# JohnLonginotto/uq

Measured on NVIDIA B200. Metric: fastq_to_uq_encode_reads_per_s, higher is better.
Workload: dtype u8

## Files before the change

uq_b200/csrc/common.cuh:

```cuda
#pragma once
#include <cuda_runtime.h>
#include <stdint.h>
#include <stdio.h>
#include <string.h>
#include <string>
#include <vector>
#include <map>
#include "../../include/uqb200.h"

#define UQB_SM_COUNT 148

struct uqb_timer_rec { const char* name; cudaEvent_t a, b; uint64_t bytes; };
struct uqb_timer_tot { uint64_t launches = 0; double ms = 0; uint64_t bytes = 0; };

struct uqb_arena {
    unsigned long long base = 0;
    uint64_t reserved = 0;
    uint64_t mapped = 0;
    uint64_t granularity = 0;
    std::map<uint64_t, uint64_t> free_by_off;
    std::map<uint64_t, uint64_t> used;
    std::vector<unsigned long long> handles;
    std::vector<std::pair<uint64_t, uint64_t>> chunks;
};
// ... 5 lines not shown
    bool own_stream = false;
    cudaStream_t copy_stream = nullptr;
    char err[512] = {0};
    uint64_t launches = 0;
    uint64_t bytes_in_use = 0;
    int sm_count = UQB_SM_COUNT;
    std::vector<const void*> copies_in_flight;
    unsigned side_ctas_per_sm = 0;
    void* pinned = nullptr;
    size_t pinned_bytes = 0;
    bool timing = false;
    std::vector<uqb_timer_rec> pending;
    std::vector<cudaEvent_t> free_events;
    std::map<std::string, uqb_timer_tot> totals;
    cudaEvent_t span_a = nullptr, span_b = nullptr;
};

struct uqb_array {
    void* d = nullptr;
    uint64_t n = 0;
    uint32_t width = 0;
    bool owned = true;
    uint64_t* key0 = nullptr;
    uint64_t nbytes() const { return n * (uint64_t)width; }
};

struct uqb_qcol {
    int64_t* val = nullptr;
    uint32_t* span = nullptr;
    uint32_t* rank = nullptr;
    uint32_t* first_occ = nullptr;
    uint8_t* dict = nullptr;
    uint64_t dict_count = 0;
    uint32_t dict_width = 0;
};

struct uqb_fastq {
    const uint8_t* d = nullptr;
    uint64_t n = 0;
    bool owned = false;
    uint64_t* line_off = nullptr;
    uint64_t n_lines = 0, n_reads = 0;
    uint64_t total_bases = 0;
    uint8_t* ref_name = nullptr;
    uint32_t ref_len = 0;
    uint64_t rbase = 0;
    uint8_t* names = nullptr;
    uint32_t name_pitch = 0;
    uint64_t names_cap = 0;
    uint64_t line_cap = 0;
    void* scan_acc = nullptr;
    bool streamed = false;
    uqb_stats* cached_stats = nullptr;
    uint32_t prefix_len = 0, suffix_len = 0, ncols = 0;
    std::vector<uqb_qcol> qcols;
};

int uqb_fail(uqb_ctx* ctx, const char* fmt, ...);

#define UQB_CUDA(expr)                                                                       \
    do {                                                                                     \
        cudaError_t _e = (expr);                                                             \
        if (_e != cudaSuccess)                                                               \
            return uqb_fail(ctx, "%s:%d %s -> %s", __FILE__, __LINE__, #expr, cudaGetErrorString(_e)); \
    } while (0)

#define UQB_TRY(expr)                                                                        \
    do {                                                                                     \
        int _r = (expr);                                                                     \
        if (_r != 0) return _r;                                                              \
    } while (0)

int uqb_dalloc(uqb_ctx* ctx, void** p, size_t nbytes);
int uqb_dfree(uqb_ctx* ctx, void* p, size_t nbytes);
int uqb_new_array(uqb_ctx* ctx, uint64_t n, uint32_t width, uqb_array** out);
int uqb_adopt_array(uqb_ctx* ctx, void* d, uint64_t n, uint32_t width, uqb_array** out);
int uqb_pinned(uqb_ctx* ctx, size_t nbytes, void** out);
int uqb_readback(uqb_ctx* ctx, void* host, const void* dev, size_t nbytes);

template <typename T>
static inline int uqb_dalloc_t(uqb_ctx* ctx, T** p, size_t count) {
    return uqb_dalloc(ctx, (void**)p, count * sizeof(T));
}

void uqb_timer_begin(uqb_ctx* ctx, const char* name, uint64_t bytes);
void uqb_timer_end(uqb_ctx* ctx);
void uqb_timer_add_bytes(uqb_ctx* ctx, uint64_t bytes);

#define UQB_LAUNCH(kernel, grid, block, smem, ...) UQB_LAUNCH_B(0, kernel, grid, block, smem, __VA_ARGS__)
#define UQB_LAUNCH_B(abytes, kernel, grid, block, smem, ...)                                 \
    do {                                                                                     \
        uqb_timer_begin(ctx, #kernel, (uint64_t)(abytes));                                   \
        kernel<<<(grid), (block), (smem), ctx->stream>>>(__VA_ARGS__);                       \
        uqb_timer_end(ctx);                                                                  \
        ctx->launches++;                                                                     \
        UQB_CUDA(cudaGetLastError());                                                        \
    } while (0)

static inline unsigned uqb_blocks(uint64_t n, unsigned per_block) {
    uint64_t b = (n + per_block - 1) / per_block;
    if (b == 0) b = 1;
    return (unsigned)b;
}

static inline unsigned uqb_grid(uqb_ctx* ctx, uint64_t n, unsigned per_block, unsigned waves = 8) {
    uint64_t need = (n + per_block - 1) / per_block;
    uint64_t cap = (uint64_t)ctx->sm_count * waves;
    if (need < 1) need = 1;
    return (unsigned)(need < cap ? need : cap);
}

#ifdef __CUDACC__
__device__ __forceinline__ unsigned lane_id() { return threadIdx.x & 31u; }

__device__ __forceinline__ uint64_t load_be64(const uint8_t* p, uint32_t avail) {
    uint64_t v = 0;
#pragma unroll
    for (int i = 0; i < 8; i++) {
        uint64_t b = (uint32_t)i < avail ? (uint64_t)__ldg(p + i) : 0ull;
        v = (v << 8) | b;
    }
    return v;
}

__device__ __forceinline__ void atomic_min_i64(int64_t* addr, int64_t v) {
    atomicMin((long long*)addr, (long long)v);
}
__device__ __forceinline__ void atomic_max_i64(int64_t* addr, int64_t v) {
    atomicMax((long long*)addr, (long long)v);
}
#endif

#define UQB_SPLIT_TILE (256 * 64)
int uqb_split_count_tiles(uqb_ctx* ctx, const uint8_t* d, uint64_t n_end, uint64_t tile0, uint64_t ntiles, uint32_t* counts);
int uqb_split_write_tiles(uqb_ctx* ctx, const uint8_t* d, uint64_t n_end, uint64_t tile0, uint64_t ntiles, uint64_t line_base,
                          const uint64_t* bases, uint64_t* line_off);
int uqb_split_set_first(uqb_ctx* ctx, uint64_t* line_off);
int uqb_copy_stream(uqb_ctx* ctx, cudaStream_t* out);
int uqb_scan_file(uqb_ctx* ctx, uqb_fastq* fq, bool* done);
int uqb_scan_release(uqb_ctx* ctx, uqb_fastq* fq);

int uqb_scan_u32(uqb_ctx* ctx, const uint32_t* d_in, uint32_t* d_out, uint64_t n, uint32_t* d_total);
int uqb_scan_u32_to_u64(uqb_ctx* ctx, const uint32_t* d_in, uint64_t* d_out, uint64_t n, uint64_t* d_total);

struct uqb_sortbuf {
    uint64_t* key[2] = {nullptr, nullptr};
    uint32_t* aux[2] = {nullptr, nullptr};
    uint32_t* val[2] = {nullptr, nullptr};
    int cur = 0;
    uint64_t cap = 0;
};
int uqb_sortbuf_alloc(uqb_ctx* ctx, uqb_sortbuf* sb, uint64_t n, bool with_aux);
int uqb_sortbuf_free(uqb_ctx* ctx, uqb_sortbuf* sb);
int uqb_radix_sort(uqb_ctx* ctx, uqb_sortbuf* sb, uint64_t n, bool use_aux, const uint64_t* key_first = nullptr);
int uqb_scatter_pairs_u32(uqb_ctx* ctx, const uint32_t* idx, const uint32_t* val, uint64_t n, uint32_t* out);

int uqb_sort_rows_impl(uqb_ctx* ctx, const uint8_t* rows, uint64_t n, uint32_t width,
                       uint32_t** d_perm, uint32_t** d_gid_sorted, uint64_t* n_unique, const uint64_t* key0 = nullptr,
                       uint64_t** sorted_keys = nullptr);
```

uq_b200/csrc/prims.cu:

```cuda
#include "common.cuh"

#define PR_THREADS 256
#define PR_ITEMS 16
#define PR_TILE (PR_THREADS * PR_ITEMS)

template <typename T>
__device__ __forceinline__ T block_exclusive_scan(T v, T* total_out) {
    __shared__ T warp_tot[PR_THREADS / 32];
    unsigned lane = lane_id(), w = threadIdx.x >> 5;
    T incl = v;
#pragma unroll
    for (int o = 1; o < 32; o <<= 1) {
        T t = __shfl_up_sync(0xffffffffu, incl, o);
        if (lane >= (unsigned)o) incl += t;
    }
    if (lane == 31) warp_tot[w] = incl;
    __syncthreads();
    T wbase = 0, tot = 0;
#pragma unroll
    for (int i = 0; i < PR_THREADS / 32; i++) {
        T t = warp_tot[i];
        if ((unsigned)i < w) wbase += t;
        tot += t;
    }
// ... 486 lines not shown
    const uint64_t tile0 = (uint64_t)tile * PR_TILE;
    const uint64_t warp0 = tile0 + (uint64_t)w * (32 * RS_ITEMS);
    const uint32_t ntile = (uint32_t)((n - tile0 < PR_TILE) ? (n - tile0) : PR_TILE);
    uint64_t key[RS_ITEMS];
    uint32_t val[RS_ITEMS];
#pragma unroll
    for (int j = 0; j < RS_ITEMS; j++) {
        const uint64_t idx = warp0 + (uint64_t)j * 32 + lane;
        key[j] = 0; val[j] = 0;
        if (idx < n) {
            key[j] = kin[idx];
            val[j] = vin ? vin[idx] : (uint32_t)idx;
        }
    }
    uint32_t rk[RS_ITEMS];
#pragma unroll
    for (int j = 0; j < RS_ITEMS; j++) {
        const uint64_t idx = warp0 + (uint64_t)j * 32 + lane;
        const bool valid = idx < n;
        uint32_t d = 256u;
        if (valid) d = (uint32_t)((key[j] >> shift) & 255ull);
        const unsigned m = __match_any_sync(0xffffffffu, d);
        const unsigned r = __popc(m & ((1u << lane) - 1u));
        const int leader = __ffs(m) - 1;
        uint32_t old = 0;
        if (valid && (int)lane == leader) {
            old = S->whist[w][d];
            S->whist[w][d] = old + __popc(m);
        }
        old = __shfl_sync(0xffffffffu, old, leader);
        rk[j] = (d << 16) | (old + r);
        if (next_shift >= 0 && valid) atomicAdd(&S->nhist[(uint32_t)((key[j] >> next_shift) & 255ull)], 1u);
        __syncwarp();
    }
    __syncthreads();
    uint32_t tot = 0, incl = 0;
    if (tid < 256) {
#pragma unroll
        for (int w2 = 0; w2 < RS_WARPS; w2++) {
            const uint32_t c = S->whist[w2][tid];
            S->whist[w2][tid] = tot;
            tot += c;
        }
        uint32_t* st = status + (uint64_t)tile * 256 + tid;
        __threadfence();
        os_st(st, (tile == 0 ? OS_FLAG_INC : OS_FLAG_AGG) | tot);
        incl = tot;
#pragma unroll
        for (int o = 1; o < 32; o <<= 1) {
            const uint32_t t = __shfl_up_sync(0xffffffffu, incl, o);
            if (lane >= (unsigned)o) incl += t;
        }
        if (lane == 31) S->wtot[w] = incl;
        if (next_shift >= 0 && S->nhist[tid]) atomicAdd(&ghist_next[tid], S->nhist[tid]);
    }
    __syncthreads();
    if (tid < 256) {
        uint32_t wb = 0;
#pragma unroll
        for (int i = 0; i < 8; i++) if ((unsigned)i < w) wb += S->wtot[i];
        const uint32_t start = wb + incl - tot;
        S->dstart[tid] = start;
        const uint32_t gh = __ldg(ghist + tid);
        uint32_t gin = gh;
#pragma unroll
        for (int o = 1; o < 32; o <<= 1) {
            const uint32_t t = __shfl_up_sync(0xffffffffu, gin, o);
            if (lane >= (unsigned)o) gin += t;
        }
        if (lane == 31) S->gtot[w] = gin;
        asm volatile("bar.sync 1, 256;" ::: "memory");
        uint32_t gb = 0;
#pragma unroll
        for (int i = 0; i < 8; i++) if ((unsigned)i < w) gb += S->gtot[i];
        const uint32_t gexcl = gb + gin - gh;
        uint32_t before = 0;
        if (tile) {
            uint32_t j = tile - 1;
            while (true) {
                uint32_t v = os_ld(status + (uint64_t)j * 256 + tid);
                while ((v & (OS_FLAG_AGG | OS_FLAG_INC)) == 0) { __nanosleep(32); v = os_ld(status + (uint64_t)j * 256 + tid); }
                before += v & OS_COUNT;
                if ((v & OS_FLAG_INC) || j == 0) break;
                j--;
            }
            __threadfence();
            os_st(status + (uint64_t)tile * 256 + tid, OS_FLAG_INC | (before + tot));
        }
        S->gbase[tid] = gexcl + before - start;
    }
    __syncthreads();
#pragma unroll
    for (int j = 0; j < RS_ITEMS; j++) {
        const uint64_t idx = warp0 + (uint64_t)j * 32 + lane;
        if (idx < n) {
            const uint32_t d = rk[j] >> 16;
            const uint32_t slot = S->dstart[d] + S->whist[w][d] + (rk[j] & 0xffffu);
            S->key[slot] = key[j];
            S->val[slot] = val[j];
        }
    }
    __syncthreads();
    for (uint32_t i = tid; i < ntile; i += RS_THREADS) {
        const uint64_t k = S->key[i];
        const uint32_t d = (uint32_t)((k >> shift) & 255ull);
        const uint32_t pos = S->gbase[d] + i;
        kout[pos] = k;
        vout[pos] = S->val[i];
    }
}

int uqb_sortbuf_alloc(uqb_ctx* ctx, uqb_sortbuf* sb, uint64_t n, bool with_aux) {
    sb->cap = n;
    sb->cur = 0;
    for (int i = 0; i < 2; i++) {
        UQB_TRY(uqb_dalloc_t(ctx, &sb->key[i], n));
        UQB_TRY(uqb_dalloc_t(ctx, &sb->val[i], n + 16));
        if (with_aux) UQB_TRY(uqb_dalloc_t(ctx, &sb->aux[i], n));
    }
    return 0;
}

int uqb_sortbuf_free(uqb_ctx* ctx, uqb_sortbuf* sb) {
    for (int i = 0; i < 2; i++) {
        UQB_TRY(uqb_dfree(ctx, sb->key[i], sb->cap * 8)); sb->key[i] = nullptr;
        UQB_TRY(uqb_dfree(ctx, sb->val[i], sb->cap * 4)); sb->val[i] = nullptr;
        if (sb->aux[i]) { UQB_TRY(uqb_dfree(ctx, sb->aux[i], sb->cap * 4)); sb->aux[i] = nullptr; }
    }
    return 0;
}

static int plan_windows(uint64_t varying, int nbits, int* shifts) {
    int cnt = 0;
    int b = 0;
    while (b < nbits) {
        if ((varying >> b) & 1ull) {
            shifts[cnt++] = b;
            b += 8;
        } else {
            b++;
        }
    }
    return cnt;
}

__global__ void __launch_bounds__(256) k_key_iota(const uint64_t* __restrict__ kin, uint64_t* __restrict__ kout, uint32_t* __restrict__ vout, uint64_t n) {
    for (uint64_t i = (uint64_t)blockIdx.x * blockDim.x + threadIdx.x; i < n; i += (uint64_t)gridDim.x * blockDim.x) { kout[i] = kin[i]; vout[i] = (uint32_t)i; }
}

#define MSD_MIN_N (1u << 20)

struct msd_counts { uint32_t nseg, nbuck, ntiles, pad; };

struct bs_stage {
    uint32_t whist[RS_WARPS][256];
    uint32_t dstart[256];
    uint32_t wtot[8];
    unsigned long long or64, and64;
    uint64_t key[PR_TILE];
    uint32_t val[PR_TILE];
};

__global__ void __launch_bounds__(RS_THREADS, 2) k_bucket_sort(const uint64_t* __restrict__ kin, const uint32_t* __restrict__ vin,
                                                              uint64_t* __restrict__ kout, uint32_t* __restrict__ vout,
                                                              const uint2* __restrict__ segs) {
    extern __shared__ __align__(16) uint8_t bs_raw[];
    bs_stage* S = reinterpret_cast<bs_stage*>(bs_raw);
    const unsigned tid = threadIdx.x, w = tid >> 5, lane = tid & 31u;
    const uint2 seg = segs[blockIdx.x];
    const uint64_t base = seg.x;
    const uint32_t m = seg.y;
    if (tid == 0) { S->or64 = 0ull; S->and64 = ~0ull; }
    __syncthreads();
    unsigned long long o64 = 0ull, a64 = ~0ull;
    for (uint32_t i = tid; i < m; i += RS_THREADS) {
        const uint64_t k = kin[base + i];
        S->key[i] = k;
        S->val[i] = vin[base + i];
        o64 |= k; a64 &= k;
    }
#pragma unroll
    for (int o = 16; o > 0; o >>= 1) {
        o64 |= __shfl_xor_sync(0xffffffffu, o64, o);
        a64 &= __shfl_xor_sync(0xffffffffu, a64, o);
    }
    if (lane == 0) { atomicOr(&S->or64, o64); atomicAnd(&S->and64, a64); }
    __syncthreads();
    uint64_t vary = S->or64 ^ S->and64;
    while (vary) {
        const int shift = __ffsll((long long)vary) - 1;
        vary = shift + 8 >= 64 ? 0ull : vary & (~0ull << (shift + 8));
        uint64_t key[RS_ITEMS];
        uint32_t val[RS_ITEMS], rk[RS_ITEMS];
#pragma unroll
        for (int j = 0; j < RS_ITEMS; j++) {
            const uint32_t i = w * (32 * RS_ITEMS) + j * 32 + lane;
            key[j] = i < m ? S->key[i] : 0ull;
            val[j] = i < m ? S->val[i] : 0u;
        }
        for (unsigned i = tid; i < RS_WARPS * 256; i += RS_THREADS) (&S->whist[0][0])[i] = 0;
        __syncthreads();
#pragma unroll
        for (int j = 0; j < RS_ITEMS; j++) {
            const uint32_t i = w * (32 * RS_ITEMS) + j * 32 + lane;
            const bool valid = i < m;
            const uint32_t d = valid ? (uint32_t)((key[j] >> shift) & 255ull) : 256u;
            const unsigned mm = __match_any_sync(0xffffffffu, d);
            const unsigned r = __popc(mm & ((1u << lane) - 1u));
            const int leader = __ffs(mm) - 1;
            uint32_t old = 0;
            if (valid && (int)lane == leader) {
                old = S->whist[w][d];
                S->whist[w][d] = old + __popc(mm);
            }
            old = __shfl_sync(0xffffffffu, old, leader);
            rk[j] = (d << 16) | (old + r);
            __syncwarp();
        }
        __syncthreads();
        uint32_t tot = 0, incl = 0;
        if (tid < 256) {
#pragma unroll
            for (int w2 = 0; w2 < RS_WARPS; w2++) {
                const uint32_t c = S->whist[w2][tid];
                S->whist[w2][tid] = tot;
                tot += c;
            }
            incl = tot;
#pragma unroll
            for (int o = 1; o < 32; o <<= 1) {
                const uint32_t t = __shfl_up_sync(0xffffffffu, incl, o);
                if (lane >= (unsigned)o) incl += t;
            }
            if (lane == 31) S->wtot[w] = incl;
        }
        __syncthreads();
        if (tid < 256) {
            uint32_t wb = 0;
#pragma unroll
            for (int i = 0; i < 8; i++) if ((unsigned)i < w) wb += S->wtot[i];
            S->dstart[tid] = wb + incl - tot;
        }
        __syncthreads();
#pragma unroll
        for (int j = 0; j < RS_ITEMS; j++) {
            const uint32_t i = w * (32 * RS_ITEMS) + j * 32 + lane;
            if (i < m) {
                const uint32_t d = rk[j] >> 16;
                const uint32_t slot = S->dstart[d] + S->whist[w][d] + (rk[j] & 0xffffu);
                S->key[slot] = key[j];
                S->val[slot] = val[j];
            }
        }
        __syncthreads();
    }
    for (uint32_t i = tid; i < m; i += RS_THREADS) {
        kout[base + i] = S->key[i];
        vout[base + i] = S->val[i];
    }
}

__global__ void __launch_bounds__(256) k_msd_plan(const uint32_t* __restrict__ goff, const msd_bucket* __restrict__ buckets, int last,
                                                 msd_counts* __restrict__ cnt, uint2* __restrict__ segs, msd_bucket* __restrict__ next,
                                                 uint32_t* __restrict__ next_tile_bucket) {
    __shared__ uint32_t st[257];
    __shared__ uint2 lseg[256], lover[256];
    __shared__ uint32_t nls, nlo, sbase, obase, t0s;
    const unsigned tid = threadIdx.x;
    const msd_bucket b = buckets[blockIdx.x];
    const uint64_t h0 = (uint64_t)b.t0 * 256;
    st[tid] = b.start + (goff[h0 + (uint64_t)tid * b.nt] - goff[h0]);
    if (tid == 0) st[256] = b.start + b.size;
    __syncthreads();
    if (last) {
        const uint32_t s = st[tid + 1] - st[tid], nch = (s + PR_TILE - 1) / PR_TILE;
        if (nch) {
            const uint32_t at = atomicAdd(&cnt->nseg, nch);
            for (uint32_t k = 0; k < nch; k++) segs[at + k] = make_uint2(st[tid] + k * PR_TILE, min((uint32_t)PR_TILE, s - k * PR_TILE));
        }
        return;
    }
    if (tid == 0) {
        uint32_t ns = 0, no = 0, cs = 0, cn = 0;
        for (int d = 0; d < 256; d++) {
            const uint32_t s = st[d + 1] - st[d];
            if (s == 0) continue;
            if (s > PR_TILE) {
                if (cn) { lseg[ns++] = make_uint2(cs, cn); cn = 0; }
                lover[no++] = make_uint2(st[d], s);
            } else {
                if (cn + s > PR_TILE) { lseg[ns++] = make_uint2(cs, cn); cn = 0; }
                if (cn == 0) cs = st[d];
                cn += s;
            }
        }
        if (cn) lseg[ns++] = make_uint2(cs, cn);
        nls = ns; nlo = no;
        sbase = ns ? atomicAdd(&cnt->nseg, ns) : 0u;
        obase = no ? atomicAdd(&cnt->nbuck, no) : 0u;
    }
    __syncthreads();
    for (uint32_t i = tid; i < nls; i += 256) segs[sbase + i] = lseg[i];
    for (uint32_t k = 0; k < nlo; k++) {
        const uint2 o = lover[k];
        const uint32_t nt = (o.y + PR_TILE - 1) / PR_TILE;
        if (tid == 0) {
            t0s = atomicAdd(&cnt->ntiles, nt);
            next[obase + k] = msd_bucket{o.x, o.y, t0s, nt};
        }
        __syncthreads();
        for (uint32_t t = tid; t < nt; t += 256) next_tile_bucket[t0s + t] = obase + k;
        __syncthreads();
    }
}

static int msd_shift(uint64_t vary, int below) {
    const uint64_t v = below >= 64 ? vary : vary & ((1ull << below) - 1);
    if (!v) return -1;
    const int hi = 63 - __builtin_clzll(v);
    return hi >= 7 ? hi - 7 : 0;
}

static int msd_sort(uqb_ctx* ctx, uqb_sortbuf* sb, uint64_t n, const uint64_t* key_first, uint64_t vary) {
    const uint32_t nblk = (uint32_t)((n + PR_TILE - 1) / PR_TILE);
    const uint64_t cap_b = n / PR_TILE + 1, cap_t = nblk + cap_b;
    const int fin = sb->cur ^ 1;
    msd_bucket* bk[2];
    uint32_t* tb[2];
    msd_counts* cnt;
    UQB_TRY(uqb_dalloc_t(ctx, &bk[0], cap_b));
    UQB_TRY(uqb_dalloc_t(ctx, &bk[1], cap_b));
    UQB_TRY(uqb_dalloc_t(ctx, &tb[0], cap_t));
    UQB_TRY(uqb_dalloc_t(ctx, &tb[1], cap_t));
    UQB_TRY(uqb_dalloc_t(ctx, &cnt, 1));
    const msd_bucket all = {0u, (uint32_t)n, 0u, nblk};
    UQB_CUDA(cudaMemcpyAsync(bk[0], &all, sizeof(all), cudaMemcpyHostToDevice, ctx->stream));
    UQB_CUDA(cudaMemsetAsync(tb[0], 0, (uint64_t)nblk * 4, ctx->stream));
    auto k_radix_hist_seg = k_radix_hist<false, true>;
    auto k_radix_scatter_seg = k_radix_scatter<false, false, true>;
    UQB_CUDA(cudaFuncSetAttribute(k_radix_scatter_seg, cudaFuncAttributeMaxDynamicSharedMemorySize, (int)sizeof(rs_stage)));
    UQB_CUDA(cudaFuncSetAttribute(k_bucket_sort, cudaFuncAttributeMaxDynamicSharedMemorySize, (int)sizeof(bs_stage)));
    uint32_t nbuck = 1, ntiles = nblk;
    uint64_t items = n;
    int c = sb->cur, shift = msd_shift(vary, 64), lv = 0;
    while (nbuck) {
        const int o = c ^ 1, nxt = msd_shift(vary, shift);
        const uint64_t* kin = (lv == 0 && key_first) ? key_first : sb->key[c];
        const uint32_t* vin = (lv == 0 && key_first) ? nullptr : sb->val[c];
        uint32_t* ghist;
        const uint64_t hist_n = (uint64_t)256 * ntiles;
        UQB_TRY(uqb_dalloc_t(ctx, &ghist, hist_n));
        UQB_LAUNCH_B((uint64_t)items * 8, k_radix_hist_seg, ntiles, PR_THREADS, 0, kin, nullptr, n, shift, ghist, 0u, tb[lv & 1], bk[lv & 1]);
        UQB_TRY(uqb_scan_u32(ctx, ghist, ghist, hist_n, nullptr));
        UQB_LAUNCH_B((uint64_t)items * 24, k_radix_scatter_seg, ntiles, RS_THREADS, sizeof(rs_stage), kin, nullptr, vin, sb->key[o], nullptr,
                     sb->val[o], n, shift, ghist, 0u, tb[lv & 1], bk[lv & 1]);
        uint2* segs;
        const uint64_t cap_s = (uint64_t)256 * nbuck + n / PR_TILE + 1;
        UQB_TRY(uqb_dalloc_t(ctx, &segs, cap_s));
        UQB_CUDA(cudaMemsetAsync(cnt, 0, sizeof(msd_counts), ctx->stream));
        UQB_LAUNCH(k_msd_plan, nbuck, 256, 0, ghist, bk[lv & 1], nxt < 0 ? 1 : 0, cnt, segs, bk[(lv + 1) & 1], tb[(lv + 1) & 1]);
        msd_counts got;
        UQB_TRY(uqb_readback(ctx, &got, cnt, sizeof(got)));
        if (got.nseg) UQB_LAUNCH_B(0, k_bucket_sort, got.nseg, RS_THREADS, sizeof(bs_stage), sb->key[o], sb->val[o], sb->key[fin], sb->val[fin], segs);
        UQB_TRY(uqb_dfree(ctx, segs, cap_s * 8));
        UQB_TRY(uqb_dfree(ctx, ghist, hist_n * 4));
        nbuck = got.nbuck;
        ntiles = got.ntiles;
        items = (uint64_t)ntiles * PR_TILE;
        c = o;
        shift = nxt;
        lv++;
    }
    sb->cur = fin;
    UQB_TRY(uqb_dfree(ctx, bk[0], cap_b * sizeof(msd_bucket)));
    UQB_TRY(uqb_dfree(ctx, bk[1], cap_b * sizeof(msd_bucket)));
    UQB_TRY(uqb_dfree(ctx, tb[0], cap_t * 4));
    UQB_TRY(uqb_dfree(ctx, tb[1], cap_t * 4));
    UQB_TRY(uqb_dfree(ctx, cnt, sizeof(msd_counts)));
    return 0;
}

int uqb_radix_sort(uqb_ctx* ctx, uqb_sortbuf* sb, uint64_t n, bool use_aux, const uint64_t* key_first) {
    if (key_first && (use_aux || n < 2)) {
        if (n) UQB_LAUNCH_B(n * 20, k_key_iota, uqb_grid(ctx, n, 256 * 8), 256, 0, key_first, sb->key[sb->cur], sb->val[sb->cur], n);
        key_first = nullptr;
    }
    if (n < 2) return 0;
    if (n >= (1ull << 32)) return uqb_fail(ctx, "radix sort: %llu items exceed the 32-bit index range", (unsigned long long)n);
    bits_summary init = {0ull, ~0ull, 0u, ~0u}, got;
    bits_summary* d_bits;
    UQB_TRY(uqb_dalloc_t(ctx, &d_bits, 1));
    UQB_CUDA(cudaMemcpyAsync(d_bits, &init, sizeof(init), cudaMemcpyHostToDevice, ctx->stream));
    UQB_LAUNCH_B(n * (use_aux ? 12 : 8), k_bits_reduce, uqb_grid(ctx, n, 256 * 8), 256, 0, key_first ? key_first : sb->key[sb->cur], use_aux ? sb->aux[sb->cur] : nullptr, n, d_bits);
    UQB_TRY(uqb_readback(ctx, &got, d_bits, sizeof(got)));
    UQB_TRY(uqb_dfree(ctx, d_bits, sizeof(bits_summary)));

    int kshift[16], ashift[8];
    int nk = plan_windows(got.or64 ^ got.and64, 64, kshift);
    int na = use_aux ? plan_windows((uint64_t)(got.or32 ^ got.and32), 32, ashift) : 0;
    if (nk + na == 0) {
        if (key_first) UQB_LAUNCH_B(n * 20, k_key_iota, uqb_grid(ctx, n, 256 * 8), 256, 0, key_first, sb->key[sb->cur], sb->val[sb->cur], n);
        return 0;
    }

    const bool has_aux = sb->aux[0] != nullptr;
    if (!use_aux && !has_aux && n >= MSD_MIN_N && nk >= 3) return msd_sort(ctx, sb, n, key_first, got.or64 ^ got.and64);
    uint32_t nblk = (uint32_t)((n + PR_TILE - 1) / PR_TILE);
    static const bool one_sweep = [] { const char* e = getenv("UQB_RADIX_ONESWEEP"); return e && e[0] == '1'; }();
    if (!use_aux && sb->aux[0] == nullptr && n < (1ull << 30) && one_sweep) {
        const uint64_t words = (uint64_t)nk * 256 + 64 + (uint64_t)nk * nblk * 256;
        uint32_t* ws;
        UQB_TRY(uqb_dalloc_t(ctx, &ws, words));
        UQB_CUDA(cudaMemsetAsync(ws, 0, words * 4, ctx->stream));
        uint32_t* gh = ws;
        unsigned int* tickets = ws + (uint64_t)nk * 256;
        uint32_t* status = ws + (uint64_t)nk * 256 + 64;
        const uint64_t* k0 = key_first ? key_first : sb->key[sb->cur];
        UQB_LAUNCH_B(n * 8, k_radix_hist_global, uqb_grid(ctx, n, PR_THREADS * 16, 8), PR_THREADS, 0, k0, n, kshift[0], gh);
        const size_t os_smem = sizeof(os_stage);
        UQB_CUDA(cudaFuncSetAttribute(k_radix_onesweep, cudaFuncAttributeMaxDynamicSharedMemorySize, (int)os_smem));
        for (int p = 0; p < nk; p++) {
            const int c = sb->cur, o = c ^ 1;
            const uint64_t* kin = (p == 0 && key_first) ? key_first : sb->key[c];
            const uint32_t* vin = (p == 0 && key_first) ? nullptr : sb->val[c];
            UQB_LAUNCH_B(n * 24, k_radix_onesweep, nblk, RS_THREADS, os_smem, kin, vin, sb->key[o], sb->val[o], n, kshift[p],
                         p + 1 < nk ? kshift[p + 1] : -1, gh + 256 * p, gh + 256 * (p + 1 < nk ? p + 1 : p),
                         status + (uint64_t)p * nblk * 256, tickets + p);
            sb->cur = o;
        }
        UQB_TRY(uqb_dfree(ctx, ws, words * 4));
        return 0;
    }
    uint32_t* ghist;
    uint64_t hist_n = (uint64_t)256 * nblk;
    UQB_TRY(uqb_dalloc_t(ctx, &ghist, hist_n));
    for (int p = 0; p < nk + na; p++) {
        bool auxd = p >= nk;
        int shift = auxd ? ashift[p - nk] : kshift[p];
        int c = sb->cur, o = c ^ 1;
        const uint64_t* kin = (p == 0 && key_first) ? key_first : sb->key[c];
        const uint32_t* vin = (p == 0 && key_first) ? nullptr : sb->val[c];
        if (auxd) UQB_LAUNCH_B(n * 4, k_radix_hist<true>, nblk, PR_THREADS, 0, kin, sb->aux[c], n, shift, ghist, nblk);
        else      UQB_LAUNCH_B(n * 8, k_radix_hist<false>, nblk, PR_THREADS, 0, kin, sb->aux[c], n, shift, ghist, nblk);
        UQB_TRY(uqb_scan_u32(ctx, ghist, ghist, hist_n, nullptr));
        auto k_radix_scatter_aux = k_radix_scatter<true, true>;
        auto k_radix_scatter_key_aux = k_radix_scatter<false, true>;
        auto k_radix_scatter_key = k_radix_scatter<false, false>;
        const size_t rs_smem = sizeof(rs_stage);
        UQB_CUDA(cudaFuncSetAttribute(k_radix_scatter_aux, cudaFuncAttributeMaxDynamicSharedMemorySize, (int)rs_smem));
        UQB_CUDA(cudaFuncSetAttribute(k_radix_scatter_key_aux, cudaFuncAttributeMaxDynamicSharedMemorySize, (int)rs_smem));
        UQB_CUDA(cudaFuncSetAttribute(k_radix_scatter_key, cudaFuncAttributeMaxDynamicSharedMemorySize, (int)rs_smem));
        if (auxd)         UQB_LAUNCH_B(n * 32, k_radix_scatter_aux, nblk, RS_THREADS, rs_smem, kin, sb->aux[c], vin, sb->key[o], sb->aux[o], sb->val[o], n, shift, ghist, nblk, nullptr, nullptr);
        else if (has_aux) UQB_LAUNCH_B(n * 32, k_radix_scatter_key_aux, nblk, RS_THREADS, rs_smem, kin, sb->aux[c], vin, sb->key[o], sb->aux[o], sb->val[o], n, shift, ghist, nblk, nullptr, nullptr);
        else              UQB_LAUNCH_B(n * 24, k_radix_scatter_key, nblk, RS_THREADS, rs_smem, kin, sb->aux[c], vin, sb->key[o], sb->aux[o], sb->val[o], n, shift, ghist, nblk, nullptr, nullptr);
        sb->cur = o;
    }
    UQB_TRY(uqb_dfree(ctx, ghist, hist_n * 4));
    return 0;
}
```

uq_b200/csrc/sort.cu:

```cuda
#include "common.cuh"

#define ST 256

__global__ void __launch_bounds__(ST) k_chunk0_keys(const uint8_t* __restrict__ rows, uint64_t n, uint32_t width,
                                                   uint64_t* __restrict__ key, uint32_t* __restrict__ val) {
    uint64_t i = (uint64_t)blockIdx.x * ST + threadIdx.x;
    if (i >= n) return;
    key[i] = load_be64(rows + i * width, width < 8 ? width : 8);
    val[i] = (uint32_t)i;
}

#define SORT_ZOFF_MIN_WIDTH 256
__global__ void __launch_bounds__(ST) k_leading_zero_bytes(const uint8_t* __restrict__ rows, uint64_t n, uint32_t width,
                                                          uint32_t* __restrict__ zoff) {
    const unsigned lane = threadIdx.x & 31u;
    const uint64_t wstride = (uint64_t)gridDim.x * (ST / 32);
    for (uint64_t i = (uint64_t)blockIdx.x * (ST / 32) + (threadIdx.x >> 5); i < n; i += wstride) {
        const uint8_t* row = rows + i * width;
        uint32_t z = width;
        const uint32_t head = (uint32_t)((16u - ((uintptr_t)row & 15u)) & 15u);
        for (uint32_t b0 = 0; b0 < head && b0 < width && z == width; b0 += 32) {
            const uint32_t b = b0 + lane;
            const bool nz = b < head && b < width && row[b] != 0;
            const unsigned m = __ballot_sync(0xffffffffu, nz);
// ... 396 lines not shown
            for (uint32_t t = 0; t < maxsz; t++) {
                const uint32_t i = gs + t;
                const bool act = multi && i < ge && i != lane;
                const unsigned di = __shfl_sync(0xffffffffu, dmask, act ? i : lane);
                if (act) {
                    unsigned m = di | dmask;
                    int c = 0;
                    while (m) {
                        const uint32_t wd = (uint32_t)__ffs((int)m) - 1u;
                        m &= m - 1u;
                        const uint32_t a = srows[i * pitch + wd], b = srows[lane * pitch + wd];
                        if (a != b) { c = a < b ? -1 : 1; break; }
                    }
                    if (c < 0 || (c == 0 && i < lane)) rank++;
                    if (c == 0 && i < lane) eq_before = true;
                }
            }
            __syncwarp();
            if (multi) {
                perm[cur + gs + rank] = r;
                if (rank > 0) head_out[cur + gs + rank] = eq_before ? 0u : 1u;
                done[cur + lane] = 1;
            }
            cur += cnt;
        }
    }
    if (lane == 0 && my_large) atomicAdd(large_rows, my_large);
}

__global__ void __launch_bounds__(ST) k_small_groups_gmem(const uint8_t* __restrict__ rows, uint32_t width, uint32_t off,
                                                         const uint32_t* __restrict__ zoff, uint32_t* __restrict__ perm, uint32_t* __restrict__ head, uint8_t* __restrict__ done,
                                                         const uint32_t* __restrict__ headpos, const uint32_t* __restrict__ d_ngroups,
                                                         unsigned long long* __restrict__ large_rows) {
    const unsigned lane = threadIdx.x & 31u, w = threadIdx.x >> 5;
    const uint32_t G = *d_ngroups;
    const uint64_t warps_total = (uint64_t)gridDim.x * (ST / 32);
    unsigned long long my_large = 0;
    for (uint64_t g0 = ((uint64_t)blockIdx.x * (ST / 32) + w) * 32; g0 < G; g0 += warps_total * 32) {
        const uint64_t g = g0 + lane;
        uint32_t start = 0, size = 0;
        if (g < G) { start = headpos[g]; size = headpos[g + 1] - start; }
        const bool fin = size < 2 || done[start];
        if (size > SG_MAX && !fin) my_large += size;
        unsigned need = __ballot_sync(0xffffffffu, size <= SG_MAX && !fin);
        while (need) {
            const int src = __ffs(need) - 1;
            need &= need - 1;
            const uint32_t s = __shfl_sync(0xffffffffu, start, src), sz = __shfl_sync(0xffffffffu, size, src);
            const uint32_t r = lane < sz ? perm[s + lane] : 0u;
            const uint32_t z = __shfl_sync(0xffffffffu, (zoff && lane < sz) ? zoff[r] : 0u, 0);
            const uint32_t rem = z + off < width ? width - z - off : 0u;
            uint32_t rank = 0;
            bool eq_before = false;
            for (uint32_t j = 0; j < sz; j++) {
                const uint32_t rj = __shfl_sync(0xffffffffu, r, j);
                if (lane < sz && j != lane) {
                    int c = 0;
                    const uint8_t* pa = rows + (uint64_t)rj * width + z + off;
                    const uint8_t* pb = rows + (uint64_t)r * width + z + off;
                    for (uint32_t i = 0; i < rem; i++) {
                        const unsigned a = __ldg(pa + i), b = __ldg(pb + i);
                        if (a != b) { c = a < b ? -1 : 1; break; }
                    }
                    if (c < 0 || (c == 0 && j < lane)) rank++;
                    if (c == 0 && j < lane) eq_before = true;
                }
            }
            __syncwarp();
            if (lane < sz) {
                perm[s + rank] = r;
                if (rank > 0) head[s + rank] = eq_before ? 0u : 1u;
                done[s + lane] = 1;
            }
            __syncwarp();
        }
    }
#pragma unroll
    for (int o = 16; o > 0; o >>= 1) my_large += __shfl_xor_sync(0xffffffffu, my_large, o);
    if (lane == 0 && my_large) atomicAdd(large_rows, my_large);
}

__global__ void __launch_bounds__(ST) k_compact_active(const uint8_t* __restrict__ rows, uint32_t width, const uint32_t* __restrict__ glcp,
                                                      const uint32_t* __restrict__ zoff, const uint32_t* __restrict__ act, const uint32_t* __restrict__ apos,
                                                      const uint32_t* __restrict__ head, const uint32_t* __restrict__ excl,
                                                      const uint32_t* __restrict__ perm, uint64_t n, uint32_t* __restrict__ pos_list,
                                                      uint64_t* __restrict__ key, uint32_t* __restrict__ aux, uint32_t* __restrict__ val) {
    uint64_t p = (uint64_t)blockIdx.x * ST + threadIdx.x;
    if (p >= n || !act[p]) return;
    uint32_t j = apos[p];
    uint32_t row = perm[p];
    pos_list[j] = (uint32_t)p;
    const uint32_t z = zoff ? zoff[row] : 0u;
    const uint32_t g = excl[p] + head[p] - 1;
    const uint32_t off = glcp[g];
    const uint32_t rem = z + off < width ? width - z - off : 0u;
    key[j] = load_be64(rows + (uint64_t)row * width + z + off, rem < 8 ? rem : 8);
    aux[j] = g;
    val[j] = row;
}

__global__ void __launch_bounds__(ST) k_write_back(const uint64_t* __restrict__ key, const uint32_t* __restrict__ aux,
                                                  const uint32_t* __restrict__ val, const uint32_t* __restrict__ pos_list, uint64_t m,
                                                  uint32_t* __restrict__ perm, uint32_t* __restrict__ head) {
    uint64_t j = (uint64_t)blockIdx.x * ST + threadIdx.x;
    if (j >= m) return;
    uint32_t p = pos_list[j];
    perm[p] = val[j];
    head[p] = (j == 0 || aux[j] != aux[j - 1] || key[j] != key[j - 1]) ? 1u : 0u;
}

__global__ void __launch_bounds__(ST) k_gid_from_scan(const uint32_t* __restrict__ head, uint32_t* __restrict__ excl_inout, uint64_t n) {
    uint64_t p = (uint64_t)blockIdx.x * ST + threadIdx.x;
    if (p >= n) return;
    excl_inout[p] = excl_inout[p] + head[p] - 1;
}

__global__ void __launch_bounds__(ST) k_iota_zero(uint32_t* __restrict__ perm, uint32_t* __restrict__ gid, uint64_t n) {
    uint64_t p = (uint64_t)blockIdx.x * ST + threadIdx.x;
    if (p >= n) return;
    perm[p] = (uint32_t)p;
    gid[p] = 0;
}

int uqb_sort_rows_impl(uqb_ctx* ctx, const uint8_t* rows, uint64_t n, uint32_t width,
                       uint32_t** d_perm, uint32_t** d_gid_sorted, uint64_t* n_unique, const uint64_t* key0, uint64_t** sorted_keys) {
    *d_perm = nullptr; *d_gid_sorted = nullptr; *n_unique = 0;
    if (sorted_keys) *sorted_keys = nullptr;
    if (n >= (1ull << 32)) return uqb_fail(ctx, "sort_rows: %llu rows exceed the 32-bit index range", (unsigned long long)n);
    uint32_t *perm = nullptr, *head, *excl;
    UQB_TRY(uqb_dalloc_t(ctx, &excl, n + 16));
    if (n == 0 || width == 0) UQB_TRY(uqb_dalloc_t(ctx, &perm, n + 16));
    if (n == 0) { *d_perm = perm; *d_gid_sorted = excl; return 0; }
    const unsigned nb = uqb_blocks(n, ST);
    if (width == 0) {
        UQB_LAUNCH(k_iota_zero, nb, ST, 0, perm, excl, n);
        *d_perm = perm; *d_gid_sorted = excl; *n_unique = 1;
        return 0;
    }
    UQB_TRY(uqb_dalloc_t(ctx, &head, n));
    uint32_t* d_tot;
    UQB_TRY(uqb_dalloc_t(ctx, &d_tot, 2));

    uint32_t* zoff = nullptr;
    if (width > SORT_ZOFF_MIN_WIDTH) {
        UQB_TRY(uqb_dalloc_t(ctx, &zoff, n));
        UQB_LAUNCH_B(n * 4, k_leading_zero_bytes, uqb_grid(ctx, n, ST / 32, 16), ST, 0, rows, n, width, zoff);
    }
    {
        uqb_sortbuf sb;
        UQB_TRY(uqb_sortbuf_alloc(ctx, &sb, n, zoff != nullptr));
        const uint64_t* kf = (!zoff && width >= 8) ? key0 : nullptr;
        if (zoff) UQB_LAUNCH_B(n * 24, k_chunk0_keys_z, nb, ST, 0, rows, n, width, zoff, sb.key[0], sb.aux[0], sb.val[0]);
        else if (!kf) UQB_LAUNCH_B(n * ((width < 8 ? width : 8) + 12), k_chunk0_keys, nb, ST, 0, rows, n, width, sb.key[0], sb.val[0]);
        UQB_TRY(uqb_radix_sort(ctx, &sb, n, zoff != nullptr, kf));
        UQB_LAUNCH(k_mark_heads, nb, ST, 0, sb.key[sb.cur], zoff ? sb.aux[sb.cur] : (const uint32_t*)nullptr, n, head);
        perm = sb.val[sb.cur];
        sb.val[sb.cur] = nullptr;
        if (sorted_keys && width <= 8 && !zoff) { *sorted_keys = sb.key[sb.cur]; sb.key[sb.cur] = nullptr; }
        UQB_TRY(uqb_sortbuf_free(ctx, &sb));
    }
    if (width > 8) {
        const uint32_t off = 8;
        uint32_t *headpos, *glcp, *act = nullptr, *apos = nullptr;
        uint8_t* done;
        unsigned long long* d_large;
        UQB_TRY(uqb_dalloc_t(ctx, &headpos, n + 1));
        UQB_TRY(uqb_dalloc_t(ctx, &glcp, n));
        UQB_TRY(uqb_dalloc_t(ctx, &done, n));
        UQB_TRY(uqb_dalloc_t(ctx, &d_large, 1));
        UQB_CUDA(cudaMemsetAsync(done, 0, n, ctx->stream));
        const uint32_t max_rounds = (width + 7) / 8 + 1;
        bool finished = false;
        if (width - off <= 128 && !zoff) {
            const uint32_t rem = width - off, pitch = (rem + 3) / 4;
            uint32_t* head2;
            UQB_TRY(uqb_dalloc_t(ctx, &head2, n));
            UQB_CUDA(cudaMemcpyAsync(head2, head, n * 4, cudaMemcpyDeviceToDevice, ctx->stream));
            UQB_CUDA(cudaMemsetAsync(d_large, 0, 8, ctx->stream));
            const size_t smem = (size_t)(ST / 32) * 32 * pitch * 4;
            const unsigned grid = uqb_grid(ctx, (n + SGP_CHUNK - 1) / SGP_CHUNK, ST / 32, 16);
            const uint64_t ab = n * ((uint64_t)rem + 13);
            if (pitch <= 8) {
                auto k_small_groups_packed_8 = k_small_groups_packed<8>;
                UQB_LAUNCH_B(ab, k_small_groups_packed_8, grid, ST, smem, rows, width, off, perm, head, head2, done, n, pitch, d_large);
            } else if (pitch <= 16) {
                auto k_small_groups_packed_16 = k_small_groups_packed<16>;
                UQB_LAUNCH_B(ab, k_small_groups_packed_16, grid, ST, smem, rows, width, off, perm, head, head2, done, n, pitch, d_large);
            } else {
                auto k_small_groups_packed_32 = k_small_groups_packed<32>;
                UQB_LAUNCH_B(ab, k_small_groups_packed_32, grid, ST, smem, rows, width, off, perm, head, head2, done, n, pitch, d_large);
            }
            UQB_TRY(uqb_dfree(ctx, head, n * 4));
            head = head2;
            unsigned long long large = 0;
            UQB_TRY(uqb_readback(ctx, &large, d_large, 8));
            finished = large == 0;
        }
        for (uint32_t round = 0; round < max_rounds && !finished; round++) {
            UQB_TRY(uqb_scan_u32(ctx, head, excl, n, d_tot));
            UQB_LAUNCH(k_headpos, nb, ST, 0, head, excl, n, headpos, glcp);
            const uint32_t rem = width - off;
            UQB_CUDA(cudaMemsetAsync(d_large, 0, 8, ctx->stream));
            const unsigned sg_grid = uqb_grid(ctx, n, ST, 16);
            if (rem <= SG_STAGE_BYTES && !zoff) {
                const uint32_t pitch = (rem + 3) / 4;
                const size_t smem = (size_t)(ST / 32) * (SG_MAX * pitch + 64) * 4;
                if (pitch <= 8) {
                    auto k_small_groups_8 = k_small_groups<8, 1>;
                    UQB_LAUNCH(k_small_groups_8, sg_grid, ST, smem, rows, width, off, perm, head, done, headpos, d_tot, pitch, d_large);
                } else if (pitch <= 16) {
                    auto k_small_groups_16 = k_small_groups<16, 1>;
                    UQB_LAUNCH(k_small_groups_16, sg_grid, ST, smem, rows, width, off, perm, head, done, headpos, d_tot, pitch, d_large);
                } else if (pitch <= 32) {
                    auto k_small_groups_32 = k_small_groups<32, 1>;
                    UQB_CUDA(cudaFuncSetAttribute(k_small_groups_32, cudaFuncAttributeMaxDynamicSharedMemorySize, (int)smem));
                    UQB_LAUNCH(k_small_groups_32, sg_grid, ST, smem, rows, width, off, perm, head, done, headpos, d_tot, pitch, d_large);
                } else {
                    auto k_small_groups_64 = k_small_groups<32, 2>;
                    UQB_CUDA(cudaFuncSetAttribute(k_small_groups_64, cudaFuncAttributeMaxDynamicSharedMemorySize, (int)smem));
                    UQB_LAUNCH(k_small_groups_64, sg_grid, ST, smem, rows, width, off, perm, head, done, headpos, d_tot, pitch, d_large);
                }
            } else {
                UQB_LAUNCH(k_small_groups_gmem, sg_grid, ST, 0, rows, width, off, zoff, perm, head, done, headpos, d_tot, d_large);
            }
            unsigned long long large = 0;
            UQB_TRY(uqb_readback(ctx, &large, d_large, 8));
            if (large == 0) break;
            const uint64_t ab_lcp = n * ((uint64_t)rem + 16);
            if (rem <= 32) {
                auto k_group_lcp_8 = k_group_lcp<8>;
                UQB_LAUNCH_B(ab_lcp, k_group_lcp_8, uqb_grid(ctx, n, ST, 16), ST, 0, rows, width, off, zoff, perm, head, excl, headpos, done, n, glcp);
            } else {
                auto k_group_lcp_32 = k_group_lcp<32>;
                UQB_LAUNCH_B(ab_lcp, k_group_lcp_32, uqb_grid(ctx, n, ST, 16), ST, 0, rows, width, off, zoff, perm, head, excl, headpos, done, n, glcp);
            }
            if (!act) {
                UQB_TRY(uqb_dalloc_t(ctx, &act, n));
                UQB_TRY(uqb_dalloc_t(ctx, &apos, n));
            }
            UQB_LAUNCH(k_active_flags, nb, ST, 0, head, excl, glcp, done, n, act);
            UQB_TRY(uqb_scan_u32(ctx, act, apos, n, d_tot + 1));
            uint32_t tot[2];
            UQB_TRY(uqb_readback(ctx, tot, d_tot, 8));
            const uint64_t m = tot[1];
            if (m == 0) break;
            uqb_sortbuf sb;
            uint32_t* pos_list;
            UQB_TRY(uqb_sortbuf_alloc(ctx, &sb, m, true));
            UQB_TRY(uqb_dalloc_t(ctx, &pos_list, m));
            UQB_LAUNCH_B(n * 8 + m * 32, k_compact_active, nb, ST, 0, rows, width, glcp, zoff, act, apos, head, excl, perm, n, pos_list, sb.key[0], sb.aux[0], sb.val[0]);
            UQB_TRY(uqb_radix_sort(ctx, &sb, m, true));
            UQB_LAUNCH_B(m * 28, k_write_back, uqb_blocks(m, ST), ST, 0, sb.key[sb.cur], sb.aux[sb.cur], sb.val[sb.cur], pos_list, m, perm, head);
            UQB_TRY(uqb_dfree(ctx, pos_list, m * 4));
            UQB_TRY(uqb_sortbuf_free(ctx, &sb));
        }
        UQB_TRY(uqb_dfree(ctx, headpos, (n + 1) * 4));
        UQB_TRY(uqb_dfree(ctx, glcp, n * 4));
        if (act) { UQB_TRY(uqb_dfree(ctx, act, n * 4)); UQB_TRY(uqb_dfree(ctx, apos, n * 4)); }
        UQB_TRY(uqb_dfree(ctx, done, n));
        UQB_TRY(uqb_dfree(ctx, d_large, 8));
    }
    if (zoff) UQB_TRY(uqb_dfree(ctx, zoff, n * 4));
    UQB_TRY(uqb_scan_u32(ctx, head, excl, n, d_tot));
    UQB_LAUNCH(k_gid_from_scan, nb, ST, 0, head, excl, n);
    uint32_t u;
    UQB_TRY(uqb_readback(ctx, &u, d_tot, 4));
    UQB_TRY(uqb_dfree(ctx, d_tot, 8));
    UQB_TRY(uqb_dfree(ctx, head, n * 4));
    *d_perm = perm;
    *d_gid_sorted = excl;
    *n_unique = u;
    return 0;
}

__global__ void __launch_bounds__(ST) k_scatter_key(const uint32_t* __restrict__ perm, const uint32_t* __restrict__ gid, uint64_t n,
                                                   uint32_t* __restrict__ key) {
    uint64_t p = (uint64_t)blockIdx.x * ST + threadIdx.x;
    if (p >= n) return;
    key[perm[p]] = gid[p];
}

__global__ void __launch_bounds__(ST) k_scatter_key_windows(const uint32_t* __restrict__ perm, const uint32_t* __restrict__ gid, uint64_t n,
                                                           uint32_t wshift, uint32_t nwin, uint32_t* __restrict__ key) {
    const uint64_t stride = (uint64_t)gridDim.x * ST * 4;
    for (uint32_t w = 0; w < nwin; w++) {
        for (uint64_t p0 = ((uint64_t)blockIdx.x * ST + threadIdx.x) * 4; p0 < n; p0 += stride) {
            if (p0 + 4 <= n) {
                const uint4 d = __ldg(reinterpret_cast<const uint4*>(perm + p0));
                if ((d.x >> wshift) == w) key[d.x] = __ldg(gid + p0);
                if ((d.y >> wshift) == w) key[d.y] = __ldg(gid + p0 + 1);
                if ((d.z >> wshift) == w) key[d.z] = __ldg(gid + p0 + 2);
                if ((d.w >> wshift) == w) key[d.w] = __ldg(gid + p0 + 3);
            } else {
                for (uint64_t p = p0; p < n; p++) { const uint32_t d = perm[p]; if ((d >> wshift) == w) key[d] = gid[p]; }
            }
        }
    }
}

static int scatter_key(uqb_ctx* ctx, const uint32_t* perm, const uint32_t* gid, uint64_t n, uint32_t* key) {
    if (n == 0) return 0;
    const uint32_t wshift = 23;
    if (n <= (3ull << wshift)) {
        UQB_LAUNCH_B(n * 12, k_scatter_key, uqb_blocks(n, ST), ST, 0, perm, gid, n, key);
        return 0;
    }
    static const bool sweeps = [] { const char* e = getenv("UQB_SCATTER_SWEEPS"); return e && e[0] == '1'; }();
    if (!sweeps) return uqb_scatter_pairs_u32(ctx, perm, gid, n, key);
    const uint32_t nwin = (uint32_t)((n + (1ull << wshift) - 1) >> wshift);
    UQB_LAUNCH_B(n * 12, k_scatter_key_windows, uqb_grid(ctx, n, ST * 4, 4), ST, 0, perm, gid, n, wshift, nwin, key);
    return 0;
// ... 484 lines not shown
```

Measured before the change: 777.4 million.

## Bin-based local sort in MSD bucket tiles and fuse head marking into sort

In the MSD bucket-sort kernel each tile now histograms keys into 2048 bins over the key span and places each key by counting smaller keys inside its bin. It falls back to the LSD digit passes only when a sum-of-squares cost estimate says the bins are too crowded. The final write can also emit segment-head flags and skip storing keys, so the separate k_mark_heads pass and the key write-back are avoided when the MSD path runs. The cost is extra shared memory, a data-dependent quadratic in-bin rank, and continuation flags packed into the segment sizes.

```diff
diff --git a/uq_b200/csrc/common.cuh b/uq_b200/csrc/common.cuh
--- a/uq_b200/csrc/common.cuh
+++ b/uq_b200/csrc/common.cuh
@@ -181,7 +181,8 @@
 };
 int uqb_sortbuf_alloc(uqb_ctx* ctx, uqb_sortbuf* sb, uint64_t n, bool with_aux);
 int uqb_sortbuf_free(uqb_ctx* ctx, uqb_sortbuf* sb);
-int uqb_radix_sort(uqb_ctx* ctx, uqb_sortbuf* sb, uint64_t n, bool use_aux, const uint64_t* key_first = nullptr);
+int uqb_radix_sort(uqb_ctx* ctx, uqb_sortbuf* sb, uint64_t n, bool use_aux, const uint64_t* key_first = nullptr,
+                   uint32_t* head_out = nullptr, bool keep_keys = true, bool* heads_written = nullptr);
 int uqb_scatter_pairs_u32(uqb_ctx* ctx, const uint32_t* idx, const uint32_t* val, uint64_t n, uint32_t* out);
 
 int uqb_sort_rows_impl(uqb_ctx* ctx, const uint8_t* rows, uint64_t n, uint32_t width,
diff --git a/uq_b200/csrc/prims.cu b/uq_b200/csrc/prims.cu
--- a/uq_b200/csrc/prims.cu
+++ b/uq_b200/csrc/prims.cu
@@ -662,46 +662,138 @@
 
 struct msd_counts { uint32_t nseg, nbuck, ntiles, pad; };
 
+#define BS_BITS 11
+#define BS_BINS (1u << BS_BITS)
+#define BS_BUDGET 16u
+#define BS_CONT 0x80000000u
+static_assert(BS_BINS == 4 * RS_THREADS, "the bin scan takes four bins per thread");
+
 struct bs_stage {
-    uint32_t whist[RS_WARPS][256];
+    union {
+        uint32_t whist[RS_WARPS][256];
+        struct { uint32_t bin[BS_BINS + 1]; uint16_t pos[PR_TILE]; } r;
+    };
     uint32_t dstart[256];
-    uint32_t wtot[8];
-    unsigned long long or64, and64;
+    uint32_t wtot[RS_WARPS];
+    unsigned long long or64, and64, min64, max64;
+    uint32_t cost, pad_;
     uint64_t key[PR_TILE];
     uint32_t val[PR_TILE];
 };
 
 __global__ void __launch_bounds__(RS_THREADS, 2) k_bucket_sort(const uint64_t* __restrict__ kin, const uint32_t* __restrict__ vin,
                                                               uint64_t* __restrict__ kout, uint32_t* __restrict__ vout,
-                                                              const uint2* __restrict__ segs) {
+                                                              uint32_t* __restrict__ head, const uint2* __restrict__ segs) {
     extern __shared__ __align__(16) uint8_t bs_raw[];
     bs_stage* S = reinterpret_cast<bs_stage*>(bs_raw);
     const unsigned tid = threadIdx.x, w = tid >> 5, lane = tid & 31u;
     const uint2 seg = segs[blockIdx.x];
     const uint64_t base = seg.x;
-    const uint32_t m = seg.y;
-    if (tid == 0) { S->or64 = 0ull; S->and64 = ~0ull; }
-    __syncthreads();
-    unsigned long long o64 = 0ull, a64 = ~0ull;
-    for (uint32_t i = tid; i < m; i += RS_THREADS) {
-        const uint64_t k = kin[base + i];
-        S->key[i] = k;
-        S->val[i] = vin[base + i];
-        o64 |= k; a64 &= k;
+    const uint32_t m = seg.y & ~BS_CONT;
+    if (tid == 0) { S->or64 = 0ull; S->and64 = ~0ull; S->min64 = ~0ull; S->max64 = 0ull; S->cost = 0u; }
+    for (uint32_t b = tid; b <= BS_BINS; b += RS_THREADS) S->r.bin[b] = 0u;
+    __syncthreads();
+    uint64_t key[RS_ITEMS];
+    uint32_t val[RS_ITEMS], loc[RS_ITEMS];
+    unsigned long long o64 = 0ull, a64 = ~0ull, mn = ~0ull, mx = 0ull;
+#pragma unroll
+    for (int j = 0; j < RS_ITEMS; j++) {
+        const uint32_t i = w * (32 * RS_ITEMS) + j * 32 + lane;
+        key[j] = 0ull; val[j] = 0u;
+        if (i < m) {
+            key[j] = kin[base + i];
+            val[j] = vin[base + i];
+            o64 |= key[j]; a64 &= key[j];
+            mn = min(mn, (unsigned long long)key[j]); mx = max(mx, (unsigned long long)key[j]);
+        }
     }
 #pragma unroll
     for (int o = 16; o > 0; o >>= 1) {
         o64 |= __shfl_xor_sync(0xffffffffu, o64, o);
         a64 &= __shfl_xor_sync(0xffffffffu, a64, o);
-    }
-    if (lane == 0) { atomicOr(&S->or64, o64); atomicAnd(&S->and64, a64); }
-    __syncthreads();
-    uint64_t vary = S->or64 ^ S->and64;
+        mn = min(mn, __shfl_xor_sync(0xffffffffu, mn, o));
+        mx = max(mx, __shfl_xor_sync(0xffffffffu, mx, o));
+    }
+    if (lane == 0) { atomicOr(&S->or64, o64); atomicAnd(&S->and64, a64); atomicMin(&S->min64, mn); atomicMax(&S->max64, mx); }
+    __syncthreads();
+    const uint64_t kmin = S->min64, span = S->max64 - kmin;
+    const int bshift = max(64 - __clzll((long long)span) - BS_BITS, 0);
+    bool lsd = false;
+    if (span) {
+#pragma unroll
+        for (int j = 0; j < RS_ITEMS; j++) {
+            const uint32_t i = w * (32 * RS_ITEMS) + j * 32 + lane;
+            if (i < m) loc[j] = atomicAdd(&S->r.bin[(uint32_t)((key[j] - kmin) >> bshift)], 1u);
+        }
+        __syncthreads();
+        uint32_t c[4], sum = 0, sq = 0;
+#pragma unroll
+        for (int q = 0; q < 4; q++) { c[q] = S->r.bin[4 * tid + q]; sum += c[q]; sq += c[q] * c[q]; }
+        uint32_t incl = sum;
+#pragma unroll
+        for (int o = 1; o < 32; o <<= 1) {
+            const uint32_t t = __shfl_up_sync(0xffffffffu, incl, o);
+            if (lane >= (unsigned)o) incl += t;
+            sq += __shfl_xor_sync(0xffffffffu, sq, o);
+        }
+        if (lane == 31) S->wtot[w] = incl;
+        if (lane == 0) atomicAdd(&S->cost, sq);
+        __syncthreads();
+        uint32_t ex = incl - sum;
+        for (unsigned i = 0; i < w; i++) ex += S->wtot[i];
+#pragma unroll
+        for (int q = 0; q < 4; q++) { S->r.bin[4 * tid + q] = ex; ex += c[q]; }
+        if (tid == 0) S->r.bin[BS_BINS] = m;
+        __syncthreads();
+        lsd = S->cost > BS_BUDGET * m;
+    }
+    if (span && !lsd) {
+#pragma unroll
+        for (int j = 0; j < RS_ITEMS; j++) {
+            const uint32_t i = w * (32 * RS_ITEMS) + j * 32 + lane;
+            if (i < m) {
+                const uint32_t slot = S->r.bin[(uint32_t)((key[j] - kmin) >> bshift)] + loc[j];
+                S->key[slot] = key[j];
+                S->val[slot] = val[j];
+                S->r.pos[slot] = (uint16_t)i;
+            }
+        }
+        __syncthreads();
+#pragma unroll
+        for (int j = 0; j < RS_ITEMS; j++) {
+            const uint32_t s = j * RS_THREADS + tid;
+            if (s < m) {
+                key[j] = S->key[s];
+                val[j] = S->val[s];
+                const uint32_t i = S->r.pos[s];
+                const uint32_t b = (uint32_t)((key[j] - kmin) >> bshift);
+                const uint32_t lo = S->r.bin[b], hi = S->r.bin[b + 1];
+                uint32_t r = lo;
+                for (uint32_t q = lo; q < hi; q++) {
+                    const uint64_t k = S->key[q];
+                    r += k < key[j] || (k == key[j] && S->r.pos[q] < i);
+                }
+                loc[j] = r;
+            }
+        }
+        __syncthreads();
+#pragma unroll
+        for (int j = 0; j < RS_ITEMS; j++) {
+            if (j * RS_THREADS + tid < m) { S->key[loc[j]] = key[j]; S->val[loc[j]] = val[j]; }
+        }
+    } else {
+#pragma unroll
+        for (int j = 0; j < RS_ITEMS; j++) {
+            const uint32_t i = w * (32 * RS_ITEMS) + j * 32 + lane;
+            if (i < m) { S->key[i] = key[j]; S->val[i] = val[j]; }
+        }
+    }
+    __syncthreads();
+    uint64_t vary = lsd ? S->or64 ^ S->and64 : 0ull;
     while (vary) {
         const int shift = __ffsll((long long)vary) - 1;
         vary = shift + 8 >= 64 ? 0ull : vary & (~0ull << (shift + 8));
-        uint64_t key[RS_ITEMS];
-        uint32_t val[RS_ITEMS], rk[RS_ITEMS];
+        uint32_t rk[RS_ITEMS];
 #pragma unroll
         for (int j = 0; j < RS_ITEMS; j++) {
             const uint32_t i = w * (32 * RS_ITEMS) + j * 32 + lane;
@@ -765,8 +857,10 @@
         __syncthreads();
     }
     for (uint32_t i = tid; i < m; i += RS_THREADS) {
-        kout[base + i] = S->key[i];
+        const uint64_t k = S->key[i];
+        if (kout) kout[base + i] = k;
         vout[base + i] = S->val[i];
+        if (head) head[base + i] = i ? (uint32_t)(k != S->key[i - 1]) : (seg.y & BS_CONT ? 0u : 1u);
     }
 }
 
@@ -786,7 +880,8 @@
         const uint32_t s = st[tid + 1] - st[tid], nch = (s + PR_TILE - 1) / PR_TILE;
         if (nch) {
             const uint32_t at = atomicAdd(&cnt->nseg, nch);
-            for (uint32_t k = 0; k < nch; k++) segs[at + k] = make_uint2(st[tid] + k * PR_TILE, min((uint32_t)PR_TILE, s - k * PR_TILE));
+            for (uint32_t k = 0; k < nch; k++)
+                segs[at + k] = make_uint2(st[tid] + k * PR_TILE, min((uint32_t)PR_TILE, s - k * PR_TILE) | (k ? BS_CONT : 0u));
         }
         return;
     }
@@ -831,7 +926,7 @@
     return hi >= 7 ? hi - 7 : 0;
 }
 
-static int msd_sort(uqb_ctx* ctx, uqb_sortbuf* sb, uint64_t n, const uint64_t* key_first, uint64_t vary) {
+static int msd_sort(uqb_ctx* ctx, uqb_sortbuf* sb, uint64_t n, const uint64_t* key_first, uint64_t vary, uint32_t* head, bool keep_keys) {
     const uint32_t nblk = (uint32_t)((n + PR_TILE - 1) / PR_TILE);
     const uint64_t cap_b = n / PR_TILE + 1, cap_t = nblk + cap_b;
     const int fin = sb->cur ^ 1;
@@ -871,7 +966,8 @@
         UQB_LAUNCH(k_msd_plan, nbuck, 256, 0, ghist, bk[lv & 1], nxt < 0 ? 1 : 0, cnt, segs, bk[(lv + 1) & 1], tb[(lv + 1) & 1]);
         msd_counts got;
         UQB_TRY(uqb_readback(ctx, &got, cnt, sizeof(got)));
-        if (got.nseg) UQB_LAUNCH_B(0, k_bucket_sort, got.nseg, RS_THREADS, sizeof(bs_stage), sb->key[o], sb->val[o], sb->key[fin], sb->val[fin], segs);
+        if (got.nseg) UQB_LAUNCH_B(0, k_bucket_sort, got.nseg, RS_THREADS, sizeof(bs_stage), sb->key[o], sb->val[o],
+                                   keep_keys ? sb->key[fin] : nullptr, sb->val[fin], head, segs);
         UQB_TRY(uqb_dfree(ctx, segs, cap_s * 8));
         UQB_TRY(uqb_dfree(ctx, ghist, hist_n * 4));
         nbuck = got.nbuck;
@@ -890,7 +986,9 @@
     return 0;
 }
 
-int uqb_radix_sort(uqb_ctx* ctx, uqb_sortbuf* sb, uint64_t n, bool use_aux, const uint64_t* key_first) {
+int uqb_radix_sort(uqb_ctx* ctx, uqb_sortbuf* sb, uint64_t n, bool use_aux, const uint64_t* key_first, uint32_t* head_out,
+                   bool keep_keys, bool* heads_written) {
+    if (heads_written) *heads_written = false;
     if (key_first && (use_aux || n < 2)) {
         if (n) UQB_LAUNCH_B(n * 20, k_key_iota, uqb_grid(ctx, n, 256 * 8), 256, 0, key_first, sb->key[sb->cur], sb->val[sb->cur], n);
         key_first = nullptr;
@@ -914,7 +1012,10 @@
     }
 
     const bool has_aux = sb->aux[0] != nullptr;
-    if (!use_aux && !has_aux && n >= MSD_MIN_N && nk >= 3) return msd_sort(ctx, sb, n, key_first, got.or64 ^ got.and64);
+    if (!use_aux && !has_aux && n >= MSD_MIN_N && nk >= 3) {
+        if (heads_written) *heads_written = head_out != nullptr;
+        return msd_sort(ctx, sb, n, key_first, got.or64 ^ got.and64, head_out, keep_keys || !head_out);
+    }
     uint32_t nblk = (uint32_t)((n + PR_TILE - 1) / PR_TILE);
     static const bool one_sweep = [] { const char* e = getenv("UQB_RADIX_ONESWEEP"); return e && e[0] == '1'; }();
     if (!use_aux && sb->aux[0] == nullptr && n < (1ull << 30) && one_sweep) {
diff --git a/uq_b200/csrc/sort.cu b/uq_b200/csrc/sort.cu
--- a/uq_b200/csrc/sort.cu
+++ b/uq_b200/csrc/sort.cu
@@ -572,11 +572,13 @@
         const uint64_t* kf = (!zoff && width >= 8) ? key0 : nullptr;
         if (zoff) UQB_LAUNCH_B(n * 24, k_chunk0_keys_z, nb, ST, 0, rows, n, width, zoff, sb.key[0], sb.aux[0], sb.val[0]);
         else if (!kf) UQB_LAUNCH_B(n * ((width < 8 ? width : 8) + 12), k_chunk0_keys, nb, ST, 0, rows, n, width, sb.key[0], sb.val[0]);
-        UQB_TRY(uqb_radix_sort(ctx, &sb, n, zoff != nullptr, kf));
-        UQB_LAUNCH(k_mark_heads, nb, ST, 0, sb.key[sb.cur], zoff ? sb.aux[sb.cur] : (const uint32_t*)nullptr, n, head);
+        const bool want_keys = sorted_keys && width <= 8 && !zoff;
+        bool heads_done = false;
+        UQB_TRY(uqb_radix_sort(ctx, &sb, n, zoff != nullptr, kf, head, want_keys, &heads_done));
+        if (!heads_done) UQB_LAUNCH(k_mark_heads, nb, ST, 0, sb.key[sb.cur], zoff ? sb.aux[sb.cur] : (const uint32_t*)nullptr, n, head);
         perm = sb.val[sb.cur];
         sb.val[sb.cur] = nullptr;
-        if (sorted_keys && width <= 8 && !zoff) { *sorted_keys = sb.key[sb.cur]; sb.key[sb.cur] = nullptr; }
+        if (want_keys) { *sorted_keys = sb.key[sb.cur]; sb.key[sb.cur] = nullptr; }
         UQB_TRY(uqb_sortbuf_free(ctx, &sb));
     }
     if (width > 8) {
```

Result: faster. 798.9 million (median of 6 runs) (+2.8%).
